# HansBambel/SmaAt-UNet

Hardware: NVIDIA H100
Metric: SmaAt-UNet fwd frames/sec @ B=32 12×288×288; depthwise % HBM roofline (higher is better)
Workload: dtype f32

## Files before the change

### include/smaat_b200.h

```cpp
#ifndef SMAAT_B200_H_
#define SMAAT_B200_H_

#include <stddef.h>
#include <stdint.h>

#ifdef __cplusplus
extern "C" {
#endif

#define SMAAT_ABI_VERSION 3

#define SMAAT_OK 0
#define SMAAT_E_BADARG (-1)
#define SMAAT_E_CUDA (-2)
#define SMAAT_E_UNSUPPORTED (-3)

#define SMAAT_PW_FP32_SIMT 0
#define SMAAT_PW_TF32 1
#define SMAAT_PW_TF32X3 2
#define SMAAT_PW_BF16 3

int smaat_abi_version(void);
const char* smaat_last_error(void);
uint64_t smaat_launch_count(void);
// ... 24 lines not shown
int smaat_dsconv_classify_eligible(const float* x0, int C0, int64_t x0_bstride, const float* x1, int C1, int64_t x1_bstride,
                                   const float* pw_w, int H, int W, int k, int Cout, int K, int mode);
int smaat_dsconv_classify_fwd(const float* x0, int C0, int64_t x0_bstride, const float* x1, int C1, int64_t x1_bstride,
                              const float* dw_w, const float* dw_b, const float* pw_w, const float* pw_w_lo,
                              const float* scale, const float* shift, const float* oc_w, const float* oc_b, int K,
                              float* logits, int64_t* classes, int B, int H, int W, int k, int Cout, int relu, int mode, void* stream);

int smaat_dsconv_cbam_eligible(const float* x0, int C0, int64_t x0_bstride, const float* x1, int C1, int64_t x1_bstride,
                               const float* pw_w, int H, int W, int k, int Cout, int mode, int with_gate, int with_pools);
int smaat_dsconv_pool_parts(int H, int W);
int smaat_dsconv_cbam_fwd(const float* x0, int C0, int64_t x0_bstride, const float* x1, int C1, int64_t x1_bstride,
                          const float* dw_w, const float* dw_b, const float* pw_w, const float* pw_w_lo,
                          const float* scale, const float* shift, float* y, int64_t y_bstride,
                          const float* gate_sc, const float* gate_sa, float* pool_sum, float* pool_max, float* pooled,
                          int B, int H, int W, int k, int Cout, int relu, int mode, void* stream);
int smaat_dsconv_maxpool_eligible(const float* x0, int C0, int64_t x0_bstride, const float* x1, int C1, int64_t x1_bstride,
                                  const float* pw_w, int H, int W, int k, int Cout, int mode);
int smaat_dsconv_maxpool_fwd(const float* x0, int C0, int64_t x0_bstride, const float* x1, int C1, int64_t x1_bstride,
                             const float* dw_w, const float* dw_b, const float* pw_w, const float* pw_w_lo,
                             const float* scale, const float* shift, float* y, int64_t y_bstride, float* pooled,
                             int B, int H, int W, int k, int Cout, int relu, int mode, void* stream);

int smaat_set_dsconv_impl(int impl);

int smaat_pw1x1_tc_eligible(const float* x, const float* w, int K, int Cout, int P);

int smaat_split_tf32(const float* src, float* hi, float* lo, int64_t n, void* stream);
int smaat_pack_bf16(const float* w, uint16_t* out, int rows, int cols, int cols_out, void* stream);

int smaat_bn_fold(const float* gamma, const float* beta, const float* rm, const float* rv,
                  const float* conv_bias, float eps, float* scale, float* shift, int C, void* stream);

int smaat_channel_stats(const float* x, double* stats, int B, int C, int P, void* stream);
int smaat_bn_finalize(const double* stats, double count, const float* gamma, const float* beta, float eps, float momentum,
                      float* running_mean, float* running_var, float* scale, float* shift,
                      float* mean_out, float* invstd_out, long long* num_batches_tracked, int C, void* stream);
int smaat_affine_act_fwd(const float* x, const float* scale, const float* shift, float* y,
                         int B, int C, int P, int act, void* stream);

int smaat_maxpool2_fwd(const float* x, float* y, int64_t N, int H, int W, void* stream);

int smaat_upsample2x_pad_fwd(const float* x, float* y, int64_t y_bstride,
                             int B, int C, int H, int W, int Ho, int Wo, void* stream);

int smaat_cbam_pool_fwd(const float* x, float* avg, float* mx, int64_t N, int P, void* stream);
int smaat_cbam_pool_maxpool_fwd(const float* x, float* avg, float* mx, float* pooled, int64_t N, int H, int W, void* stream);
// ... 129 lines not shown
```

### smaat_unet_b200/_lib.py

```python
from __future__ import annotations

import ctypes as C
import os

_HERE = os.path.dirname(os.path.abspath(__file__))
LIB_PATH = os.path.join(_HERE, "libsmaat_b200.so")

_p = C.c_void_p
_i = C.c_int
_l = C.c_int64
_f = C.c_float

SIGNATURES = {
    "smaat_dw3x3_fwd": [_p, _i, _l, _p, _i, _l, _p, _p, _p, _p, _p, _i, _i, _i, _i, _i, _p],
    "smaat_pw1x1_fwd": [_p, _p, _p, _p, _p, _p, _l, _p, _i, _i, _i, _i, _i, _i, _p],
    "smaat_pw1x1_tc_eligible": [_p, _p, _i, _i, _i],
    "smaat_dsconv_eligible": [_p, _i, _l, _p, _i, _l, _p, _i, _i, _i, _i],
    "smaat_dsconv_eligible2": [_p, _i, _l, _p, _i, _l, _p, _i, _i, _i, _i, _i],
    "smaat_set_dsconv_impl": [_i],
    "smaat_dsconv_fwd": [_p, _i, _l, _p, _i, _l, _p, _p, _p, _p, _p, _p, _p, _l, _p, _i, _i, _i, _i, _i, _i, _i, _p],
    "smaat_dsconv_outconv_fwd": [_p, _i, _l, _p, _i, _l, _p, _p, _p, _p, _p, _p, _p, _p, _p, _i, _i, _i, _i, _i, _i, _i, _p],
    "smaat_dsconv_classify_eligible": [_p, _i, _l, _p, _i, _l, _p, _i, _i, _i, _i, _i, _i],
    "smaat_dsconv_classify_fwd": [_p, _i, _l, _p, _i, _l, _p, _p, _p, _p, _p, _p, _p, _p, _i, _p, _p, _i, _i, _i, _i, _i, _i, _i, _p],
    "smaat_dsconv_cbam_eligible": [_p, _i, _l, _p, _i, _l, _p, _i, _i, _i, _i, _i, _i, _i],
    "smaat_dsconv_pool_parts": [_i, _i],
    "smaat_dsconv_maxpool_eligible": [_p, _i, _l, _p, _i, _l, _p, _i, _i, _i, _i, _i],
    "smaat_dsconv_maxpool_fwd": [_p, _i, _l, _p, _i, _l, _p, _p, _p, _p, _p, _p, _p, _l, _p, _i, _i, _i, _i, _i, _i, _i, _p],
    "smaat_dsconv_cbam_fwd": [_p, _i, _l, _p, _i, _l, _p, _p, _p, _p, _p, _p, _p, _l, _p, _p, _p, _p, _p, _i, _i, _i, _i, _i, _i, _i, _p],
    "smaat_split_tf32": [_p, _p, _p, _l, _p],
    "smaat_pack_bf16": [_p, _p, _i, _i, _i, _p],
    "smaat_bn_fold": [_p, _p, _p, _p, _p, _f, _p, _p, _i, _p],
    "smaat_channel_stats": [_p, _p, _i, _i, _i, _p],
    "smaat_bn_finalize": [_p, C.c_double, _p, _p, _f, _f, _p, _p, _p, _p, _p, _p, _p, _i, _p],
    "smaat_affine_act_fwd": [_p, _p, _p, _p, _i, _i, _i, _i, _p],
    "smaat_maxpool2_fwd": [_p, _p, _l, _i, _i, _p],
    "smaat_upsample2x_pad_fwd": [_p, _p, _l, _i, _i, _i, _i, _i, _i, _p],
    "smaat_cbam_pool_fwd": [_p, _p, _p, _l, _i, _p],
    "smaat_cbam_pool_maxpool_fwd": [_p, _p, _p, _p, _l, _i, _i, _p],
    "smaat_cbam_mlp_fwd": [_p, _p, _p, _p, _p, _p, _p, _i, _i, _i, _p],
    "smaat_cbam_reduce_fwd": [_p, _p, _p, _i, _i, _i, _p],
    "smaat_cbam_gate_fwd": [_p, _p, _p, _p, _p, _i, _i, _i, _i, _p],
    "smaat_cbam_scale_fwd": [_p, _p, _p, _p, _l, _i, _i, _i, _p],
# ... 94 lines not shown
```

### smaat_unet_b200/csrc/dsconv_fused.cu

```cuda
#include <stdlib.h>

#include <type_traits>

#include "tc_common.cuh"

namespace smaat {

struct DsParams {
  const float* dw_w;
  const float* dw_b;
  const float* scale;
  const float* shift;
  float* y;
  int64_t y_bstride;
  double* stats;
  const float* oc_w;
  const float* oc_b;
  float* oc_y;
  const float* gate_sc;
  float* pool_sum;
  float* pool_max;
  float* pooled;
  int pooled_bf16;
  int npart;
  int ncls;
  int64_t* cls;
  int C0, C1, H, W, Cout, relu, K;
  int tiles_x, tiles_y, npass, total_tiles, nchunks;
};

constexpr int DS_MAX_CLASSES = 32;

template <int N_TILE, int KPL, int PW, Prec P, bool A_SMEM, typename TA = float>
struct DsCfg {
  static constexpr bool X3 = P == Prec::TF32X3;
  static constexpr int ESZ = (int)sizeof(TA);
  static_assert(ESZ == 4 || (P == Prec::BF16 && KPL != 4), "bf16 activations: the bf16 register-form instances, k = 1, 2");
  static_assert(P != Prec::BF16 || !A_SMEM, "BF16: register A form only");
  static constexpr int PH = TC_BM / PW;
  static constexpr int XM = 16 / ESZ;
  static constexpr int BW = PW + 2 * XM, BH = PH + 2;
  static constexpr int CC = TC_BK / KPL;
  static constexpr int IN_BYTES = CC * BH * BW * ESZ;
  static constexpr int A_BYTES = TC_BM * TC_BK * 4;
  static constexpr int B_BYTES = N_TILE * TC_BK * (P == Prec::BF16 ? 2 : 4);
  static constexpr int AST_BYTES = (X3 && A_SMEM ? 2 : 1) * A_BYTES;
  static constexpr int BST_BYTES = (X3 ? 2 : 1) * B_BYTES;
  static constexpr int OFF_ALO = A_BYTES;
  static constexpr int OFF_BLO = B_BYTES;
  static constexpr int NG = N_TILE > 64 ? 1 : 2;
  static constexpr int AS = X3 ? (A_SMEM ? (N_TILE > 64 ? 2 : 3) : 2 + NG) : 4;
  static constexpr int BS = X3 ? (A_SMEM && N_TILE > 64 ? 2 : 3) : 4;
  static constexpr int AFF_N = 512;
  static constexpr int BAR_BYTES = 512;
  static constexpr int FREE = 224 * 1024 - 1024 - BAR_BYTES - 3 * AFF_N * 4 - AS * AST_BYTES - BS * BST_BYTES;
  static constexpr int ST_BOX = 32 * 64 * ESZ;
  static constexpr int ST_WANT = 2;
  static constexpr int ST_BUFS = (FREE - 2 * ST_WANT * ST_BOX) / IN_BYTES >= 2 ? ST_WANT
                                 : (FREE - 2 * ST_BOX) / IN_BYTES >= 2     ? 1
                                                                           : 0;
  static constexpr int ST_BYTES = 2 * ST_BUFS * ST_BOX;
  static_assert(ST_BUFS > 0 || (FREE - 2 * ST_BOX) / IN_BYTES < 2, "staging falls back only where one buffer does not fit");
  static constexpr int SA_TX = BH * BW * 4;
  static constexpr int SA_BYTES = (SA_TX + 127) / 128 * 128;
  static constexpr int CLS_MIN = 21 * (N_TILE + 1) * 4;
  static constexpr int RING_CLS = (FREE - ST_BYTES + 3 * 1024 - CLS_MIN) / 1024 * 1024;
  static constexpr int IS_FIT = (RING_CLS < FREE - ST_BYTES ? RING_CLS : FREE - ST_BYTES) / (IN_BYTES + SA_BYTES);
  static constexpr int IS = IS_FIT > 8 ? 8 : IS_FIT;
  static_assert(IS * (IN_BYTES + SA_BYTES) + ST_BYTES <= FREE, "gate boxes fit beside the input ring");
  static constexpr int OFF_SA = IS * IN_BYTES;
  static constexpr int OFF_A = ((OFF_SA + IS * SA_BYTES + 1023) / 1024) * 1024;
  static constexpr int OFF_BR = OFF_A + AS * AST_BYTES;
  static constexpr int OFF_ST = OFF_BR + BS * BST_BYTES;
  static constexpr int OFF_BAR = OFF_ST + ST_BYTES;
  static_assert((IS * NG + IS + 2 * AS + 2 * BS) * 8 <= BAR_BYTES, "barrier block");
  static constexpr int TOTAL = OFF_BAR + BAR_BYTES + 3 * AFF_N * 4 + 1024;
  static constexpr int OFF_CLS = OFF_BAR + BAR_BYTES + 3 * AFF_N * 4;
  static constexpr int CLS_FIT = (227 * 1024 - TOTAL) / ((N_TILE + 1) * 4);
  static constexpr int MAX_CLASSES = CLS_FIT < DS_MAX_CLASSES ? CLS_FIT : DS_MAX_CLASSES;
  static constexpr int CLS_SMEM = MAX_CLASSES * (N_TILE + 1) * 4;
  static_assert(MAX_CLASSES >= 21, "the class weights of a 21-class model fit beside the rings");
  static_assert(TOTAL + CLS_SMEM <= 227 * 1024, "the class weights take no shared memory from the rings");
  static constexpr uint32_t B_TX = BST_BYTES;
  static constexpr int PROD_WARP = 12;
  static constexpr int THREADS = 384 + 128 * NG;
  static constexpr int REGS_LAUNCH = (65536 / THREADS) / 8 * 8;
  static constexpr int REGS_TMA = 24;
  static constexpr int REGS_PROD = N_TILE > 64 ? 104 : REGS_LAUNCH;
  static constexpr int REGS_MMA = ((THREADS / 128 * REGS_LAUNCH - REGS_TMA - NG * REGS_PROD) / 2) / 8 * 8;
  static constexpr int REGS_SUM = REGS_TMA + 2 * REGS_MMA + NG * REGS_PROD;
  static_assert(REGS_SUM <= THREADS / 128 * REGS_LAUNCH && REGS_MMA >= REGS_LAUNCH, "register budget");
  static constexpr int KS = (X3 && N_TILE == 64) ? 2 : TC_BK / 8;
  static_assert(IS >= 2, "input ring");
  static_assert(NG <= AS, "phase-parity barriers");
  static_assert(IN_BYTES % 128 == 0, "TMA destination alignment");
  static_assert(TOTAL <= 227 * 1024, "shared memory budget");
};

__device__ __forceinline__ void tma_store_4d(const CUtensorMap* m, uint32_t src, int c0, int c1, int c2, int c3) {
  asm volatile("cp.async.bulk.tensor.4d.global.shared::cta.bulk_group [%0, {%2, %3, %4, %5}], [%1];" ::"l"(
                   reinterpret_cast<uint64_t>(m)),
               "r"(src), "r"(c0), "r"(c1), "r"(c2), "r"(c3)
               : "memory");
}
__device__ __forceinline__ void bulk_commit() { asm volatile("cp.async.bulk.commit_group;" ::: "memory"); }
template <int N>
__device__ __forceinline__ void bulk_wait_read() { asm volatile("cp.async.bulk.wait_group.read %0;" ::"n"(N) : "memory"); }
__device__ __forceinline__ void bulk_wait_all() { asm volatile("cp.async.bulk.wait_group 0;" ::: "memory"); }
__device__ __forceinline__ void wg_sync(int id) { asm volatile("bar.sync %0, 128;" ::"r"(id) : "memory"); }

__device__ __forceinline__ void quad_transpose(float (&v)[4], int q) {
  const bool h1 = q & 2, h0 = q & 1;
#pragma unroll
  for (int e = 0; e < 2; ++e) {
    const float r = __shfl_xor_sync(0xffffffffu, h1 ? v[e] : v[e + 2], 8);
    if (h1) v[e] = r; else v[e + 2] = r;
  }
#pragma unroll
  for (int e = 0; e < 4; e += 2) {
    const float r = __shfl_xor_sync(0xffffffffu, h0 ? v[e] : v[e + 1], 4);
    if (h0) v[e] = r; else v[e + 1] = r;
  }
}

template <int N_TILE, int KPL, int PW, Prec PREC, bool A_SMEM, typename TA = float>
__device__ __forceinline__ void dsconv_body(const CUtensorMap& map_in0, const CUtensorMap& map_in1, const CUtensorMap& map_w,
                                            const CUtensorMap& map_wlo, const CUtensorMap& map_y, const CUtensorMap& map_sa,
                                            const DsParams& p) {
  using L = DsCfg<N_TILE, KPL, PW, PREC, A_SMEM, TA>;
  constexpr bool X3 = L::X3;
  constexpr bool BA = L::ESZ == 2;
  constexpr int PH = L::PH, BW = L::BW, BH = L::BH, CC = L::CC, IS = L::IS, AS = L::AS, BS = L::BS;
  extern __shared__ __align__(1024) unsigned char smem_dyn[];
  unsigned char* smem = smem_dyn + ((1024u - (smem_u32(smem_dyn) & 1023u)) & 1023u);
  unsigned char* a_base = smem + L::OFF_A;
  unsigned char* b_base = smem + L::OFF_BR;
  uint64_t* bars = reinterpret_cast<uint64_t*>(smem + L::OFF_BAR);
  uint64_t* in_full = bars;
  uint64_t* in_empty = in_full + IS * L::NG;
  uint64_t* a_full = in_empty + IS;
  uint64_t* a_empty = a_full + AS;
  uint64_t* b_full = a_empty + AS;
  uint64_t* b_empty = b_full + BS;
  float* aff = reinterpret_cast<float*>(smem + L::OFF_BAR + L::BAR_BYTES);

  const int warp = __shfl_sync(0xffffffffu, (int)(threadIdx.x >> 5), 0);
  const int lane = threadIdx.x & 31;
  const int nch = p.nchunks;
  const int tiles_per_img = p.tiles_x * p.tiles_y * p.npass;
  auto decode = [&](int tile, int& b, int& ty, int& tx, int& np) {
    b = tile / tiles_per_img;
    int t2 = tile - b * tiles_per_img;
    np = t2 % p.npass;
    t2 /= p.npass;
    ty = t2 / p.tiles_x;
    tx = t2 - ty * p.tiles_x;
  };

  if (warp == 0 && lane == 0) {
    tma_prefetch_desc(&map_in0);
    tma_prefetch_desc(&map_in1);
    tma_prefetch_desc(&map_w);
    if (X3) tma_prefetch_desc(&map_wlo);
    if (L::ST_BUFS && !p.oc_y) tma_prefetch_desc(&map_y);
    if (p.gate_sc) tma_prefetch_desc(&map_sa);
    for (int s = 0; s < IS; ++s) {
      for (int g = 0; g < L::NG; ++g) mbar_init(&in_full[s * L::NG + g], 1);
      mbar_init(&in_empty[s], 128);
    }
    for (int s = 0; s < AS; ++s) {
      mbar_init(&a_full[s], 128);
      mbar_init(&a_empty[s], 8);
    }
    for (int s = 0; s < BS; ++s) {
      mbar_init(&b_full[s], 1);
      mbar_init(&b_empty[s], 8);
    }
    fence_barrier_init();
  }
  for (int c = threadIdx.x; c < L::AFF_N; c += blockDim.x) {
    aff[c] = (c < p.Cout && p.scale) ? __ldg(p.scale + c) : 1.f;
    aff[L::AFF_N + c] = (c < p.Cout && p.shift) ? __ldg(p.shift + c) : 0.f;
    aff[2 * L::AFF_N + c] = (c < p.Cout && p.oc_w) ? __ldg(p.oc_w + c) : 0.f;
  }
  float* cls_w = reinterpret_cast<float*>(smem + L::OFF_CLS);
  float* cls_b = cls_w + L::MAX_CLASSES * N_TILE;
  if (p.ncls) {
    for (int i = threadIdx.x; i < p.ncls * N_TILE; i += blockDim.x) {
      const int cl = i / N_TILE, c = i - cl * N_TILE;
      cls_w[i] = c < p.Cout ? __ldg(p.oc_w + (int64_t)cl * p.Cout + c) : 0.f;
    }
    for (int cl = threadIdx.x; cl < p.ncls; cl += blockDim.x) cls_b[cl] = p.oc_b ? __ldg(p.oc_b + cl) : 0.f;
  }
  __syncthreads();

  if (warp < 4) {
    regs_dealloc<L::REGS_TMA>();
    if (warp == 0 && lane == 0) {
      uint32_t gc = 0;
      for (int tile = blockIdx.x; tile < p.total_tiles; tile += gridDim.x) {
        int b, ty, tx, np;
        decode(tile, b, ty, tx, np);
        const int x0 = tx * PW, y0 = ty * PH;
        for (int i = 0; i < nch; ++i, ++gc) {
          const int s = gc % IS;
          mbar_wait(&in_empty[s], ((gc / IS) & 1u) ^ 1u);
          uint64_t* full = &in_full[s * L::NG + (int)(gc % (uint32_t)L::NG)];
          const int cb = i * CC;
          const bool gated = p.gate_sc && cb < p.C0;
          mbar_arrive_expect_tx(full, L::IN_BYTES + (gated ? L::SA_TX : 0));
          if (gated) tma_load_3d(smem + L::OFF_SA + s * L::SA_BYTES, &map_sa, full, x0 - L::XM, y0 - 1, b);
          const CUtensorMap* m = (cb < p.C0) ? &map_in0 : &map_in1;
          const int cc = (cb < p.C0) ? cb : cb - p.C0;
          asm volatile(
              "cp.async.bulk.tensor.4d.shared::cluster.global.mbarrier::complete_tx::bytes [%0], [%1, {%3, %4, %5, %6}], [%2];" ::
                  "r"(smem_u32(smem + s * L::IN_BYTES)),
              "l"(reinterpret_cast<uint64_t>(m)), "r"(smem_u32(full)), "r"(x0 - L::XM), "r"(y0 - 1), "r"(cc), "r"(b)
              : "memory");
        }
      }
    }
    if (warp == 1 && lane == 0) {
      uint32_t gc = 0;
      for (int tile = blockIdx.x; tile < p.total_tiles; tile += gridDim.x) {
        int b, ty, tx, np;
        decode(tile, b, ty, tx, np);
        for (int i = 0; i < nch; ++i, ++gc) {
          const int sb = gc % BS;
          mbar_wait(&b_empty[sb], ((gc / BS) & 1u) ^ 1u);
          mbar_arrive_expect_tx(&b_full[sb], L::B_TX);
// ... 13 lines not shown
    const int m1 = A_SMEM ? m0 + 8 : tc_row_pixel(wg, wq, 1, g);
    const float act_lo = p.relu ? 0.f : -INFINITY;
    const int64_t P = (int64_t)p.H * p.W;
    constexpr int SW_MASK = PW == 32 ? 7 : 3;
    const int quad = g & 3, slot = quad ^ (t & 2);
    const int st_ch = 2 * t + (slot & 1);
    const int st_px = ((slot & 2) ? m1 : m0) - quad - 64 * wg;
    const uint32_t st_a0 = (uint32_t)(st_ch * 64 * L::ESZ + st_px * L::ESZ);
    const uint32_t st_off = BA ? st_a0 : st_a0 ^ (((st_a0 >> 7) & SW_MASK) << 4);
    const uint32_t st_base = smem_u32(smem + L::OFF_ST) + (uint32_t)(wg * L::ST_BUFS * L::ST_BOX);
    const bool st_leader = (threadIdx.x & 127) == 0;
    uint32_t st_n = 0;
    uint32_t gc = 0;
    for (int tile = blockIdx.x; tile < p.total_tiles; tile += gridDim.x) {
      int b, ty, tx, np;
      decode(tile, b, ty, tx, np);
      float acc[N_TILE / 2];
#pragma unroll
      for (int i = 0; i < N_TILE / 2; ++i) acc[i] = 0.f;
      auto release = [&](uint32_t c) {
        __syncwarp();
        if (lane == 0) {
          mbar_arrive(&a_empty[c % AS]);
          mbar_arrive(&b_empty[c % BS]);
        }
      };
      auto wait_stages = [&](const unsigned char*& ast, uint64_t& bd, uint64_t& bl) {
        const int sa = gc % AS, sb = gc % BS;
        mbar_wait(&a_full[sa], (gc / AS) & 1u);
        mbar_wait(&b_full[sb], (gc / BS) & 1u);
        ast = a_base + sa * L::AST_BYTES;
        bd = make_b_desc<PREC>(smem_u32(b_base + sb * L::BST_BYTES));
        bl = make_kmajor_desc(smem_u32(b_base + sb * L::BST_BYTES + L::OFF_BLO));
      };
      if (A_SMEM) {
        for (int i = 0; i < nch; ++i, ++gc) {
          const unsigned char* ast;
          uint64_t bd0, bl0;
          wait_stages(ast, bd0, bl0);
          const uint32_t a_addr = smem_u32(ast) + (uint32_t)(wg * 64 * 128);
          const uint64_t ad0 = make_kmajor_desc(a_addr), al0 = make_kmajor_desc(a_addr + L::OFF_ALO);
          wgmma_fence();
#pragma unroll
          for (int kk = 0; kk < TC_BK / 8; ++kk) {
            Wgmma<N_TILE>::ss(acc, ad0 + (uint64_t)(2 * kk), bd0 + (uint64_t)(2 * kk), 1u);
            if (X3) {
// ... 232 lines not shown
              if (v1) st_act(yc + o1, fmaxf(fmaf(acc[4 * j + 2 + e], sc, sh), act_lo));
            }
          }
        }
      }
    }
    if (L::ST_BUFS && st_leader) bulk_wait_all();
    return;
  }

  {
    if (L::REGS_PROD < L::REGS_LAUNCH) regs_dealloc<L::REGS_PROD>();
    const int g = (warp - L::PROD_WARP) >> 2;
    const int t = threadIdx.x - 32 * L::PROD_WARP - 128 * g;
    const int Cin = p.C0 + p.C1;
    constexpr int KH = KPL == 4 ? 2 : KPL, NT = CC * 8;
    const int kr0 = KH == KPL ? 0 : t / NT * KH;
    const float* dw_w = p.dw_w + kr0 * 9;
    const float* dw_b = p.dw_b ? p.dw_b + kr0 : nullptr;
    uint32_t gc = 0, iph = 0;
    for (int tile = blockIdx.x; tile < p.total_tiles; tile += gridDim.x) {
      const int b = tile / tiles_per_img;
      for (int i = 0; i < nch; ++i, ++gc) {
        if ((int)(gc % (uint32_t)L::NG) != g) continue;
        const int s = gc % IS;
        const bool gated = p.gate_sc && i * CC < p.C0;
        auto task_base = [&](int task) { return KH == KPL ? task : task & (NT - 1); };
        float wr[KH][9], br[KH], gsc = 0.f;
        auto task_channel = [&](int task) { return (PW == 32) ? (task >> 3) : (((task >> 4) << 1) | ((task >> 2) & 1)); };
        auto load_weights = [&](int task) {
          const int gch = i * CC + task_channel(task_base(task));
          const bool chv = gch < Cin;
#pragma unroll
          for (int kk = 0; kk < KH; ++kk) {
            const int gk = gch * KPL + kk;
#pragma unroll
            for (int w9 = 0; w9 < 9; ++w9) wr[kk][w9] = chv ? __ldg(dw_w + (int64_t)gk * 9 + w9) : 0.f;
            br[kk] = (chv && dw_b) ? __ldg(dw_b + gk) : 0.f;
          }
          if (gated) gsc = gch < p.C0 ? __ldg(p.gate_sc + (int64_t)b * p.C0 + gch) : 0.f;
        };
        load_weights(t);
        mbar_wait(&in_full[s * L::NG + g], (iph >> s) & 1u);
        iph ^= 1u << s;
        const int sa = gc % AS;
        mbar_wait(&a_empty[sa], ((gc / AS) & 1u) ^ 1u);
        unsigned char* my_op = a_base + sa * L::AST_BYTES;
        const TA* in_stage = reinterpret_cast<const TA*>(smem + s * L::IN_BYTES);
// ... 56 lines not shown
                  a = fmaf(wr[kk][0], w0[j], a); a = fmaf(wr[kk][1], w0[j + 1], a); a = fmaf(wr[kk][2], w0[j + 2], a);
                  a = fmaf(wr[kk][3], w1[j], a); a = fmaf(wr[kk][4], w1[j + 1], a); a = fmaf(wr[kk][5], w1[j + 2], a);
                  a = fmaf(wr[kk][6], w2[j], a); a = fmaf(wr[kk][7], w2[j + 1], a); a = fmaf(wr[kk][8], w2[j + 2], a);
                  o4[j] = a;
                }
                if (A_SMEM) {
                  const int kr = ci * KPL + kr0 + kk;
#pragma unroll
                  for (int j = 0; j < 4; ++j) {
                    const uint32_t off = kmajor_offset(m + j, kr);
                    const float h = X3 ? tf32_hi(o4[j]) : o4[j];
                    *reinterpret_cast<float*>(my_op + off) = h;
                    if (X3) *reinterpret_cast<float*>(my_op + L::OFF_ALO + off) = o4[j] - h;
                  }
                  continue;
                }
                *reinterpret_cast<float4*>(my_op + a_tile_offset(ci * KPL + kr0 + kk, m)) = make_float4(o4[0], o4[1], o4[2], o4[3]);
              }
            }
          }
        };
        if (gated) stencil(std::true_type{}); else stencil(std::false_type{});
        if (A_SMEM) fence_proxy_async_smem();
        mbar_arrive(&a_full[sa]);
        mbar_arrive(&in_empty[s]);
      }
    }
  }
}

__host__ __device__ constexpr Prec tf32_prec(bool x3) { return x3 ? Prec::TF32X3 : Prec::TF32; }

template <int N_TILE, int KPL, int PW, bool X3, bool A_SMEM>
__global__ void __launch_bounds__(DsCfg<N_TILE, KPL, PW, tf32_prec(X3), A_SMEM>::THREADS, 1)
    dsconv_fused_kernel(const __grid_constant__ CUtensorMap map_in0, const __grid_constant__ CUtensorMap map_in1,
                        const __grid_constant__ CUtensorMap map_w, const __grid_constant__ CUtensorMap map_wlo,
                        const __grid_constant__ CUtensorMap map_y, const __grid_constant__ CUtensorMap map_sa,
                        const DsParams p) {
  dsconv_body<N_TILE, KPL, PW, tf32_prec(X3), A_SMEM>(map_in0, map_in1, map_w, map_wlo, map_y, map_sa, p);
}

template <int N_TILE, int PW, bool X3>
__global__ void __launch_bounds__(DsCfg<N_TILE, 4, PW, tf32_prec(X3), false>::THREADS, 1)
    dsconv_kpl4_kernel(const __grid_constant__ CUtensorMap map_in0, const __grid_constant__ CUtensorMap map_in1,
                       const __grid_constant__ CUtensorMap map_w, const __grid_constant__ CUtensorMap map_wlo,
                       const __grid_constant__ CUtensorMap map_y, const __grid_constant__ CUtensorMap map_sa,
                       const DsParams p) {
  dsconv_body<N_TILE, 4, PW, tf32_prec(X3), false>(map_in0, map_in1, map_w, map_wlo, map_y, map_sa, p);
}

template <int N_TILE, int KPL, int PW>
__global__ void __launch_bounds__(DsCfg<N_TILE, KPL, PW, Prec::BF16, false>::THREADS, 1)
    dsconv_bf16_kernel(const __grid_constant__ CUtensorMap map_in0, const __grid_constant__ CUtensorMap map_in1,
                       const __grid_constant__ CUtensorMap map_w, const __grid_constant__ CUtensorMap map_wlo,
                       const __grid_constant__ CUtensorMap map_y, const __grid_constant__ CUtensorMap map_sa,
                       const DsParams p) {
  dsconv_body<N_TILE, KPL, PW, Prec::BF16, false>(map_in0, map_in1, map_w, map_wlo, map_y, map_sa, p);
}

template <int N_TILE, int KPL, int PW>
__global__ void __launch_bounds__(DsCfg<N_TILE, KPL, PW, Prec::BF16, false, uint16_t>::THREADS, 1)
    dsconv_bf16act_kernel(const __grid_constant__ CUtensorMap map_in0, const __grid_constant__ CUtensorMap map_in1,
                          const __grid_constant__ CUtensorMap map_w, const __grid_constant__ CUtensorMap map_wlo,
                          const __grid_constant__ CUtensorMap map_y, const __grid_constant__ CUtensorMap map_sa,
                          const DsParams p) {
  dsconv_body<N_TILE, KPL, PW, Prec::BF16, false, uint16_t>(map_in0, map_in1, map_w, map_wlo, map_y, map_sa, p);
}

template <int N_TILE, int KPL, int PW, Prec P, bool A_SMEM, typename TA = float>
static auto ds_kernel() {
  static_assert(KPL == 1 || KPL == 2 || (KPL == 4 && !A_SMEM), "fused DS conv instances: k = 1, 2 (both A forms), 4 (register form)");
  if constexpr (sizeof(TA) == 2) return dsconv_bf16act_kernel<N_TILE, KPL, PW>;
  else if constexpr (P == Prec::BF16) return dsconv_bf16_kernel<N_TILE, KPL, PW>;
  else if constexpr (KPL == 4) return dsconv_kpl4_kernel<N_TILE, PW, P == Prec::TF32X3>;
  else return dsconv_fused_kernel<N_TILE, KPL, PW, P == Prec::TF32X3, A_SMEM>;
}

template <int N_TILE, int KPL, int PW, Prec P, bool A_SMEM, typename TA = float>
static int launch_ds(const CUtensorMap& m0, const CUtensorMap& m1, const CUtensorMap& mw, const CUtensorMap& mwl,
                     const CUtensorMap& my, const CUtensorMap& msa, DsParams p, int B, cudaStream_t st) {
  using L = DsCfg<N_TILE, KPL, PW, P, A_SMEM, TA>;
  auto kern = ds_kernel<N_TILE, KPL, PW, P, A_SMEM, TA>();
  if (p.pooled && !L::ST_BUFS) return fail(SMAAT_E_UNSUPPORTED, "dsconv: the CBAM pools and the max-pool need the staged epilogue");
  if (p.ncls > L::MAX_CLASSES)
    return fail(SMAAT_E_UNSUPPORTED, "dsconv+classify: %d classes, this instance keeps the weights of at most %d", p.ncls, L::MAX_CLASSES);
  static std::atomic<uint64_t> attr_mask{0};
  if (first_use_on_device(attr_mask)) {
    cudaError_t e = cudaFuncSetAttribute(kern, cudaFuncAttributeMaxDynamicSharedMemorySize, L::TOTAL + L::CLS_SMEM);
    if (e != cudaSuccess)
      return fail(SMAAT_E_CUDA, "dsconv: smem attribute (%d B): %s", L::TOTAL + L::CLS_SMEM, cudaGetErrorString(e));
    int r = check_reg_budget((const void*)kern, L::THREADS, L::REGS_SUM, "dsconv");
    if (r) return r;
  }
  p.tiles_x = ceil_div(p.W, PW);
  p.tiles_y = ceil_div(p.H, L::PH);
  p.npass = ceil_div(p.Cout, N_TILE);
  const int64_t total = (int64_t)B * p.tiles_x * p.tiles_y * p.npass;
  SMAAT_REQUIRE(total < (1ll << 31), "dsconv: too many tiles");
  p.total_tiles = (int)total;
  p.nchunks = ceil_div(p.C0 + p.C1, L::CC);
  p.npart = 2 * p.tiles_x * p.tiles_y;
  const int grid = p.total_tiles < num_sms() ? p.total_tiles : num_sms();
  kern<<<grid, L::THREADS, L::TOTAL + (p.ncls ? L::CLS_SMEM : 0), st>>>(m0, m1, mw, mwl, my, msa, p);
  SMAAT_LAUNCH_CHECK("smaat_dsconv_fwd");
  return SMAAT_OK;
}

static int pick_pw(int H, int W) {
  double best = 1e9;
  int pw = 0;
  const int cand[2] = {32, 16};
  for (int i = 0; i < 2; ++i) {
    const int c = cand[i], ph = TC_BM / c;
    const double waste = ((double)ceil_div(W, c) * c / W) * ((double)ceil_div(H, ph) * ph / H);
    if (waste < best - 1e-9) {
      best = waste;
      pw = c;
    }
  }
  return best <= 1.35 ? pw : 0;
}

static int ds_impl();

static bool ds_eligible(const float* x0, int C0, int64_t bs0, const float* x1, int C1, int64_t bs1, const float* pw_w,
                        const float* pw_w_lo, const float* y, int64_t y_bstride, int H, int W, int k, int Cout, bool stats,
                        bool outconv, bool bf16 = false, bool bact = false) {
  if (k != 1 && k != 2 && !(k == 4 && ds_impl() != 1)) return false;
// ... 41 lines not shown
}

static std::atomic<int> g_ds_impl{-1};
static int ds_impl() {
  int v = g_ds_impl.load(std::memory_order_relaxed);
  if (v < 0) {
    const char* e = getenv("SMAAT_DS_IMPL");
    v = e ? atoi(e) : 0;
    if (v < 0 || v > 2) v = 0;
    g_ds_impl.store(v, std::memory_order_relaxed);
  }
  return v;
}

}

using namespace smaat;

extern "C" int smaat_set_dsconv_impl(int impl) {
  SMAAT_REQUIRE(impl >= 0 && impl <= 2, "set_dsconv_impl: 0 = auto, 1 = A operand from shared memory, 2 = A operand from registers");
  g_ds_impl.store(impl, std::memory_order_relaxed);
  return SMAAT_OK;
}

extern "C" int smaat_dsconv_eligible2(const float* x0, int C0, int64_t x0_bstride, const float* x1, int C1, int64_t x1_bstride,
                                      const float* pw_w, int H, int W, int k, int Cout, int with_stats) {
  return ds_eligible(x0, C0, x0_bstride, x1, C1, x1_bstride, pw_w, nullptr, nullptr, 0, H, W, k, Cout, with_stats != 0, false) ? 1
                                                                                                                                : 0;
}

extern "C" int smaat_dsconv_eligible(const float* x0, int C0, int64_t x0_bstride, const float* x1, int C1, int64_t x1_bstride,
                                     const float* pw_w, int H, int W, int k, int Cout) {
  return smaat_dsconv_eligible2(x0, C0, x0_bstride, x1, C1, x1_bstride, pw_w, H, W, k, Cout, 0);
}

extern "C" int smaat_dsconv_cbam_eligible(const float* x0, int C0, int64_t x0_bstride, const float* x1, int C1, int64_t x1_bstride,
                                          const float* pw_w, int H, int W, int k, int Cout, int mode, int with_gate, int with_pools) {
  if (mode != SMAAT_PW_TF32 && mode != SMAAT_PW_TF32X3 && mode != SMAAT_PW_BF16) return 0;
  if (!ds_eligible(x0, C0, x0_bstride, x1, C1, x1_bstride, pw_w, nullptr, nullptr, 0, H, W, k, Cout, false, false,
                   mode == SMAAT_PW_BF16))
    return 0;
  (void)with_gate;
  if (with_pools && !ds_staged(Cout > 64 ? 128 : 64, k, pick_pw(H, W), mode, ds_impl() == 1)) return 0;
  return 1;
}

// ... 93 lines not shown
    const uint64_t str[3] = {0, (uint64_t)W * 4, (uint64_t)H * W * 4};
    const uint32_t sbox[3] = {(uint32_t)(pw + 2 * xm), (uint32_t)(ph + 2), 1u};
    int r = make_tmap_f32(&msa, gate_sa, 3, dims, str, sbox, CU_TENSOR_MAP_SWIZZLE_NONE, "dsconv(gate sa)");
    if (r) return r;
  }
  DsParams p;
  p.dw_w = dw_w; p.dw_b = dw_b; p.scale = scale; p.shift = shift; p.y = y; p.y_bstride = y_bstride; p.stats = stats;
  p.oc_w = oc_w; p.oc_b = oc_b; p.oc_y = oc_y; p.ncls = ncls; p.cls = cls;
  p.gate_sc = gate_sc; p.pool_sum = pool_sum; p.pool_max = pool_max; p.pooled = pooled; p.pooled_bf16 = pooled_bf16; p.npart = 0;
  p.C0 = C0; p.C1 = C1; p.H = H; p.W = W; p.Cout = Cout; p.relu = relu; p.K = K;
  p.tiles_x = p.tiles_y = p.npass = p.total_tiles = p.nchunks = 0;

#define DS_DISPATCH(NT, KP, PWv)                                                                           \
  if (bact) return launch_ds<NT, KP, PWv, Prec::BF16, false, uint16_t>(m0, m1, mw, mwl, my, msa, p, B, st);         \
  if (bf16) return launch_ds<NT, KP, PWv, Prec::BF16, false>(m0, m1, mw, mwl, my, msa, p, B, st);                    \
  return x3 ? (a_smem ? launch_ds<NT, KP, PWv, Prec::TF32X3, true>(m0, m1, mw, mwl, my, msa, p, B, st)               \
                      : launch_ds<NT, KP, PWv, Prec::TF32X3, false>(m0, m1, mw, mwl, my, msa, p, B, st))             \
            : (a_smem ? launch_ds<NT, KP, PWv, Prec::TF32, true>(m0, m1, mw, mwl, my, msa, p, B, st)                 \
                      : launch_ds<NT, KP, PWv, Prec::TF32, false>(m0, m1, mw, mwl, my, msa, p, B, st))
#define DS_DISPATCH4(NT, PWv)                                                                                  \
  if (bf16) return launch_ds<NT, 4, PWv, Prec::BF16, false>(m0, m1, mw, mwl, my, msa, p, B, st);                  \
  return x3 ? launch_ds<NT, 4, PWv, Prec::TF32X3, false>(m0, m1, mw, mwl, my, msa, p, B, st)                  \
            : launch_ds<NT, 4, PWv, Prec::TF32, false>(m0, m1, mw, mwl, my, msa, p, B, st)
  if (n_tile == 64) {
    if (k == 4)      { if (pw == 32) { DS_DISPATCH4(64, 32); } else { DS_DISPATCH4(64, 16); } }
    else if (k == 2) { if (pw == 32) { DS_DISPATCH(64, 2, 32); } else { DS_DISPATCH(64, 2, 16); } }
    else             { if (pw == 32) { DS_DISPATCH(64, 1, 32); } else { DS_DISPATCH(64, 1, 16); } }
  } else {
    if (k == 4)      { if (pw == 32) { DS_DISPATCH4(128, 32); } else { DS_DISPATCH4(128, 16); } }
    else if (k == 2) { if (pw == 32) { DS_DISPATCH(128, 2, 32); } else { DS_DISPATCH(128, 2, 16); } }
    else             { if (pw == 32) { DS_DISPATCH(128, 1, 32); } else { DS_DISPATCH(128, 1, 16); } }
  }
#undef DS_DISPATCH4
#undef DS_DISPATCH
}

extern "C" int smaat_dsconv_fwd(const float* x0, int C0, int64_t x0_bstride, const float* x1, int C1, int64_t x1_bstride,
                                const float* dw_w, const float* dw_b, const float* pw_w, const float* pw_w_lo,
                                const float* scale, const float* shift, float* y, int64_t y_bstride, double* stats, int B, int H,
                                int W, int k, int Cout, int relu, int mode, void* stream) {
  SMAAT_REQUIRE(y, "dsconv: null output");
  return dsconv_run(x0, C0, x0_bstride, x1, C1, x1_bstride, dw_w, dw_b, pw_w, pw_w_lo, scale, shift, y, y_bstride, stats, nullptr,
                    nullptr, nullptr, 0, nullptr, nullptr, nullptr, nullptr, nullptr, nullptr, B, H, W, k, Cout, relu, mode, stream);
}

extern "C" int smaat_dsconv_outconv_fwd(const float* x0, int C0, int64_t x0_bstride, const float* x1, int C1, int64_t x1_bstride,
                                        const float* dw_w, const float* dw_b, const float* pw_w, const float* pw_w_lo,
                                        const float* scale, const float* shift, const float* oc_w, const float* oc_b,
                                        float* logits, int B, int H, int W, int k, int Cout, int relu, int mode, void* stream) {
  SMAAT_REQUIRE(oc_w && logits, "dsconv+outconv: null pointer");
  return dsconv_run(x0, C0, x0_bstride, x1, C1, x1_bstride, dw_w, dw_b, pw_w, pw_w_lo, scale, shift, nullptr, 0, nullptr, oc_w, oc_b,
                    logits, 0, nullptr, nullptr, nullptr, nullptr, nullptr, nullptr, B, H, W, k, Cout, relu, mode, stream);
}

extern "C" int smaat_dsconv_classify_eligible(const float* x0, int C0, int64_t x0_bstride, const float* x1, int C1, int64_t x1_bstride,
// ... 117 lines not shown
```

### smaat_unet_b200/ops.py

```python
from __future__ import annotations

import contextlib
import ctypes as C
import gc
import os

import torch

from . import _lib

PW_MODES = {"fp32": 0, "tf32": 1, "tf32x3": 2, "bf16": 3}
_pw_mode = os.environ.get("SMAAT_PW_MODE", "tf32x3")
assert _pw_mode in PW_MODES, f"SMAAT_PW_MODE must be one of {list(PW_MODES)}"


def set_pointwise_mode(mode: str) -> None:
    global _pw_mode
    if mode not in PW_MODES:
        raise ValueError(f"pointwise mode must be one of {list(PW_MODES)}")
    _pw_mode = mode


def get_pointwise_mode() -> str:
    return _pw_mode
# ... 167 lines not shown
        ybs = Cout * P
    else:
        out, ybs = _nchw_bstride(out, "out")
    mode = mode or _pw_mode
    m = PW_MODES[mode]
    if m != 0 and (not tc_eligible(x, w2d) or (Cout > 512 and (scale is not None or shift is not None))):
        m = 0
    w2d, wlo = weight_operands(w2d, m, w_split)
    _call(f"smaat_pw1x1_fwd[K{K}_N{Cout}_P{P}]", 4 * B * P * (K + Cout) + 4 * K * Cout, 2 * B * P * K * Cout, _lib.load().smaat_pw1x1_fwd, _ptr(x), _ptr(w2d), _ptr(wlo), _ptr(scale), _ptr(shift), _ptr(out), ybs, _ptr(stats),
                                           B, K, Cout, P, int(bool(relu)), m, _stream())
    return out


_fuse_ds = os.environ.get("SMAAT_FUSE_DS", "1") != "0"


def set_fused_dsconv(enabled: bool) -> None:
    global _fuse_ds
    _fuse_ds = bool(enabled)


def set_dsconv_impl(impl: str) -> None:
    _lib.check(_lib.load().smaat_set_dsconv_impl({"auto": 0, "smem": 1, "regs": 2}[impl]), "smaat_set_dsconv_impl")


def dsconv_takes(x, x1, pw_weight, k, mode=None, stats=False) -> bool:
    mode = mode or _pw_mode
    if not _fuse_ds or PW_MODES[mode] == 0:
        return False
    x, bs0, x1, C1, bs1 = _concat_operands(x, x1)
    w2d = _pw_matrix(pw_weight)
    lib = _lib.load()
    args = (_ptr(x), x.shape[1], bs0, _ptr(x1), C1, bs1, _ptr(w2d), x.shape[2], x.shape[3], k, w2d.shape[0])
    if not lib.smaat_dsconv_eligible2(*args, int(bool(stats))):
        return False
    return PW_MODES[mode] != 3 or bool(lib.smaat_dsconv_cbam_eligible(*args, 3, 0, 0))


def dsconv_cbam_takes(x, x1, pw_weight, k, gate=False, pools=False, mode=None) -> bool:
    mode = mode or _pw_mode
    if not _fuse_ds or PW_MODES[mode] == 0:
        return False
    x, bs0, x1, C1, bs1 = _concat_operands(x, x1)
    w2d = _pw_matrix(pw_weight)
    return bool(_lib.load().smaat_dsconv_cbam_eligible(_ptr(x), x.shape[1], bs0, _ptr(x1), C1, bs1, _ptr(w2d), x.shape[2], x.shape[3], k,
                                                       w2d.shape[0], PW_MODES[mode], int(bool(gate)), int(bool(pools))))
# ... 645 lines not shown
```

Before: 2709.

## Split depthwise stencil work across 2-CTA clusters sharing A tiles via DSMEM

Measured after the change: 2767, median of 6. +2.1%, better.

```diff
diff --git a/include/smaat_b200.h b/include/smaat_b200.h
--- a/include/smaat_b200.h
+++ b/include/smaat_b200.h
@@ -70,6 +70,9 @@
                              int B, int H, int W, int k, int Cout, int relu, int mode, void* stream);
 
 int smaat_set_dsconv_impl(int impl);
+
+int smaat_set_dsconv_pair(int on);
+int smaat_dsconv_pair_clusters(void);
 
 int smaat_pw1x1_tc_eligible(const float* x, const float* w, int K, int Cout, int P);
 
diff --git a/smaat_unet_b200/_lib.py b/smaat_unet_b200/_lib.py
--- a/smaat_unet_b200/_lib.py
+++ b/smaat_unet_b200/_lib.py
@@ -18,6 +18,8 @@
     "smaat_dsconv_eligible": [_p, _i, _l, _p, _i, _l, _p, _i, _i, _i, _i],
     "smaat_dsconv_eligible2": [_p, _i, _l, _p, _i, _l, _p, _i, _i, _i, _i, _i],
     "smaat_set_dsconv_impl": [_i],
+    "smaat_set_dsconv_pair": [_i],
+    "smaat_dsconv_pair_clusters": [],
     "smaat_dsconv_fwd": [_p, _i, _l, _p, _i, _l, _p, _p, _p, _p, _p, _p, _p, _l, _p, _i, _i, _i, _i, _i, _i, _i, _p],
     "smaat_dsconv_outconv_fwd": [_p, _i, _l, _p, _i, _l, _p, _p, _p, _p, _p, _p, _p, _p, _p, _i, _i, _i, _i, _i, _i, _i, _p],
     "smaat_dsconv_classify_eligible": [_p, _i, _l, _p, _i, _l, _p, _i, _i, _i, _i, _i, _i],
diff --git a/smaat_unet_b200/csrc/dsconv_fused.cu b/smaat_unet_b200/csrc/dsconv_fused.cu
--- a/smaat_unet_b200/csrc/dsconv_fused.cu
+++ b/smaat_unet_b200/csrc/dsconv_fused.cu
@@ -31,7 +31,7 @@
 
 constexpr int DS_MAX_CLASSES = 32;
 
-template <int N_TILE, int KPL, int PW, Prec P, bool A_SMEM, typename TA = float>
+template <int N_TILE, int KPL, int PW, Prec P, bool A_SMEM, typename TA = float, int CL = 1>
 struct DsCfg {
   static constexpr bool X3 = P == Prec::TF32X3;
   static constexpr int ESZ = (int)sizeof(TA);
@@ -49,7 +49,7 @@
   static constexpr int OFF_ALO = A_BYTES;
   static constexpr int OFF_BLO = B_BYTES;
   static constexpr int NG = N_TILE > 64 ? 1 : 2;
-  static constexpr int AS = X3 ? (A_SMEM ? (N_TILE > 64 ? 2 : 3) : 2 + NG) : 4;
+  static constexpr int AS = X3 ? (A_SMEM ? (N_TILE > 64 ? 2 : 3) : 2 + (CL > 1 && KPL == 2 ? CL : 1) * NG) : 4;
   static constexpr int BS = X3 ? (A_SMEM && N_TILE > 64 ? 2 : 3) : 4;
   static constexpr int AFF_N = 512;
   static constexpr int BAR_BYTES = 512;
@@ -93,6 +93,7 @@
   static constexpr int KS = (X3 && N_TILE == 64) ? 2 : TC_BK / 8;
   static_assert(IS >= 2, "input ring");
   static_assert(NG <= AS, "phase-parity barriers");
+  static constexpr bool PAIRABLE = N_TILE == 128 && !A_SMEM && ESZ == 4 && KPL != 4 && P != Prec::BF16 && 2 * NG <= AS;
   static_assert(IN_BYTES % 128 == 0, "TMA destination alignment");
   static_assert(TOTAL <= 227 * 1024, "shared memory budget");
 };
@@ -109,6 +110,31 @@
 __device__ __forceinline__ void bulk_wait_all() { asm volatile("cp.async.bulk.wait_group 0;" ::: "memory"); }
 __device__ __forceinline__ void wg_sync(int id) { asm volatile("bar.sync %0, 128;" ::"r"(id) : "memory"); }
 
+__device__ __forceinline__ uint32_t cluster_rank() {
+  uint32_t r;
+  asm volatile("mov.u32 %0, %%cluster_ctarank;" : "=r"(r));
+  return r;
+}
+__device__ __forceinline__ void cluster_sync() {
+  asm volatile("barrier.cluster.arrive.release;\n\tbarrier.cluster.wait.acquire;" ::: "memory");
+}
+__device__ __forceinline__ uint32_t cluster_addr(uint32_t a, uint32_t rank) {
+  uint32_t r;
+  asm volatile("mapa.shared::cluster.u32 %0, %1, %2;" : "=r"(r) : "r"(a), "r"(rank));
+  return r;
+}
+__device__ __forceinline__ void mbar_arrive_remote(uint32_t bar) {
+  asm volatile("mbarrier.arrive.shared::cluster.b64 _, [%0];" ::"r"(bar) : "memory");
+}
+__device__ __forceinline__ void mbar_arrive_expect_tx_remote(uint32_t bar, uint32_t bytes) {
+  asm volatile("mbarrier.arrive.expect_tx.shared::cluster.b64 _, [%0], %1;" ::"r"(bar), "r"(bytes) : "memory");
+}
+__device__ __forceinline__ void bulk_copy_to_peer(uint32_t dst, uint32_t src, uint32_t bytes, uint32_t bar) {
+  asm volatile("cp.async.bulk.shared::cluster.shared::cta.mbarrier::complete_tx::bytes [%0], [%1], %2, [%3];" ::"r"(dst), "r"(src),
+               "r"(bytes), "r"(bar)
+               : "memory");
+}
+
 __device__ __forceinline__ void quad_transpose(float (&v)[4], int q) {
   const bool h1 = q & 2, h0 = q & 1;
 #pragma unroll
@@ -123,11 +149,12 @@
   }
 }
 
-template <int N_TILE, int KPL, int PW, Prec PREC, bool A_SMEM, typename TA = float>
+template <int N_TILE, int KPL, int PW, Prec PREC, bool A_SMEM, typename TA = float, int CL = 1>
 __device__ __forceinline__ void dsconv_body(const CUtensorMap& map_in0, const CUtensorMap& map_in1, const CUtensorMap& map_w,
                                             const CUtensorMap& map_wlo, const CUtensorMap& map_y, const CUtensorMap& map_sa,
                                             const DsParams& p) {
-  using L = DsCfg<N_TILE, KPL, PW, PREC, A_SMEM, TA>;
+  using L = DsCfg<N_TILE, KPL, PW, PREC, A_SMEM, TA, CL>;
+  static_assert(CL == 1 || (CL == 2 && L::PAIRABLE), "CTA pairs: the N_TILE 128 register-form fp32 instances, k = 1, 2");
   constexpr bool X3 = L::X3;
   constexpr bool BA = L::ESZ == 2;
   constexpr int PH = L::PH, BW = L::BW, BH = L::BH, CC = L::CC, IS = L::IS, AS = L::AS, BS = L::BS;
@@ -147,6 +174,7 @@
   const int warp = __shfl_sync(0xffffffffu, (int)(threadIdx.x >> 5), 0);
   const int lane = threadIdx.x & 31;
   const int nch = p.nchunks;
+  const uint32_t rank = CL > 1 ? cluster_rank() : 0u, peer = rank ^ 1u;
   const int tiles_per_img = p.tiles_x * p.tiles_y * p.npass;
   auto decode = [&](int tile, int& b, int& ty, int& tx, int& np) {
     b = tile / tiles_per_img;
@@ -169,8 +197,8 @@
       mbar_init(&in_empty[s], 128);
     }
     for (int s = 0; s < AS; ++s) {
-      mbar_init(&a_full[s], 128);
-      mbar_init(&a_empty[s], 8);
+      mbar_init(&a_full[s], CL > 1 ? 1 : 128);
+      mbar_init(&a_empty[s], 8 * CL);
     }
     for (int s = 0; s < BS; ++s) {
       mbar_init(&b_full[s], 1);
@@ -193,6 +221,7 @@
     for (int cl = threadIdx.x; cl < p.ncls; cl += blockDim.x) cls_b[cl] = p.oc_b ? __ldg(p.oc_b + cl) : 0.f;
   }
   __syncthreads();
+  if (CL > 1) cluster_sync();
 
   if (warp < 4) {
     regs_dealloc<L::REGS_TMA>();
@@ -203,9 +232,11 @@
         decode(tile, b, ty, tx, np);
         const int x0 = tx * PW, y0 = ty * PH;
         for (int i = 0; i < nch; ++i, ++gc) {
-          const int s = gc % IS;
-          mbar_wait(&in_empty[s], ((gc / IS) & 1u) ^ 1u);
-          uint64_t* full = &in_full[s * L::NG + (int)(gc % (uint32_t)L::NG)];
+          if (CL > 1 && gc % CL != rank) continue;
+          const uint32_t f = gc / CL;
+          const int s = f % IS;
+          mbar_wait(&in_empty[s], ((f / IS) & 1u) ^ 1u);
+          uint64_t* full = &in_full[s * L::NG + (int)(f % (uint32_t)L::NG)];
           const int cb = i * CC;
           const bool gated = p.gate_sc && cb < p.C0;
           mbar_arrive_expect_tx(full, L::IN_BYTES + (gated ? L::SA_TX : 0));
@@ -265,6 +296,7 @@
         __syncwarp();
         if (lane == 0) {
           mbar_arrive(&a_empty[c % AS]);
+          if (CL > 1) mbar_arrive_remote(cluster_addr(smem_u32(&a_empty[c % AS]), peer));
           mbar_arrive(&b_empty[c % BS]);
         }
       };
@@ -543,8 +575,10 @@
     for (int tile = blockIdx.x; tile < p.total_tiles; tile += gridDim.x) {
       const int b = tile / tiles_per_img;
       for (int i = 0; i < nch; ++i, ++gc) {
-        if ((int)(gc % (uint32_t)L::NG) != g) continue;
-        const int s = gc % IS;
+        if (CL > 1 && gc % CL != rank) continue;
+        const uint32_t f = gc / CL;
+        if ((int)(f % (uint32_t)L::NG) != g) continue;
+        const int s = f % IS;
         const bool gated = p.gate_sc && i * CC < p.C0;
         auto task_base = [&](int task) { return KH == KPL ? task : task & (NT - 1); };
         float wr[KH][9], br[KH], gsc = 0.f;
@@ -647,7 +681,18 @@
         };
         if (gated) stencil(std::true_type{}); else stencil(std::false_type{});
         if (A_SMEM) fence_proxy_async_smem();
-        mbar_arrive(&a_full[sa]);
+        if constexpr (CL > 1) {
+          fence_proxy_async_smem();
+          asm volatile("bar.sync 4, 128;" ::: "memory");
+          if (t == 0) {
+            mbar_arrive(&a_full[sa]);
+            const uint32_t rbar = cluster_addr(smem_u32(&a_full[sa]), peer);
+            mbar_arrive_expect_tx_remote(rbar, L::A_BYTES);
+            bulk_copy_to_peer(cluster_addr(smem_u32(my_op), peer), smem_u32(my_op), L::A_BYTES, rbar);
+          }
+        } else {
+          mbar_arrive(&a_full[sa]);
+        }
         mbar_arrive(&in_empty[s]);
       }
     }
@@ -665,6 +710,16 @@
   dsconv_body<N_TILE, KPL, PW, tf32_prec(X3), A_SMEM>(map_in0, map_in1, map_w, map_wlo, map_y, map_sa, p);
 }
 
+template <int KPL, int PW, bool X3>
+__global__ void __launch_bounds__(DsCfg<128, KPL, PW, tf32_prec(X3), false>::THREADS, 1)
+    dsconv_pair_kernel(const __grid_constant__ CUtensorMap map_in0, const __grid_constant__ CUtensorMap map_in1,
+                       const __grid_constant__ CUtensorMap map_w, const __grid_constant__ CUtensorMap map_wlo,
+                       const __grid_constant__ CUtensorMap map_y, const __grid_constant__ CUtensorMap map_sa,
+                       const DsParams p) {
+  dsconv_body<128, KPL, PW, tf32_prec(X3), false, float, 2>(map_in0, map_in1, map_w, map_wlo, map_y, map_sa, p);
+  cluster_sync();
+}
+
 template <int N_TILE, int PW, bool X3>
 __global__ void __launch_bounds__(DsCfg<N_TILE, 4, PW, tf32_prec(X3), false>::THREADS, 1)
     dsconv_kpl4_kernel(const __grid_constant__ CUtensorMap map_in0, const __grid_constant__ CUtensorMap map_in1,
@@ -692,20 +747,23 @@
   dsconv_body<N_TILE, KPL, PW, Prec::BF16, false, uint16_t>(map_in0, map_in1, map_w, map_wlo, map_y, map_sa, p);
 }
 
-template <int N_TILE, int KPL, int PW, Prec P, bool A_SMEM, typename TA = float>
+template <int N_TILE, int KPL, int PW, Prec P, bool A_SMEM, typename TA = float, int CL = 1>
 static auto ds_kernel() {
   static_assert(KPL == 1 || KPL == 2 || (KPL == 4 && !A_SMEM), "fused DS conv instances: k = 1, 2 (both A forms), 4 (register form)");
-  if constexpr (sizeof(TA) == 2) return dsconv_bf16act_kernel<N_TILE, KPL, PW>;
+  if constexpr (CL == 2) return dsconv_pair_kernel<KPL, PW, P == Prec::TF32X3>;
+  else if constexpr (sizeof(TA) == 2) return dsconv_bf16act_kernel<N_TILE, KPL, PW>;
   else if constexpr (P == Prec::BF16) return dsconv_bf16_kernel<N_TILE, KPL, PW>;
   else if constexpr (KPL == 4) return dsconv_kpl4_kernel<N_TILE, PW, P == Prec::TF32X3>;
   else return dsconv_fused_kernel<N_TILE, KPL, PW, P == Prec::TF32X3, A_SMEM>;
 }
 
-template <int N_TILE, int KPL, int PW, Prec P, bool A_SMEM, typename TA = float>
+static std::atomic<int> g_ds_pairs_resident{0};
+
+template <int N_TILE, int KPL, int PW, Prec P, bool A_SMEM, typename TA = float, int CL = 1>
 static int launch_ds(const CUtensorMap& m0, const CUtensorMap& m1, const CUtensorMap& mw, const CUtensorMap& mwl,
                      const CUtensorMap& my, const CUtensorMap& msa, DsParams p, int B, cudaStream_t st) {
-  using L = DsCfg<N_TILE, KPL, PW, P, A_SMEM, TA>;
-  auto kern = ds_kernel<N_TILE, KPL, PW, P, A_SMEM, TA>();
+  using L = DsCfg<N_TILE, KPL, PW, P, A_SMEM, TA, CL>;
+  auto kern = ds_kernel<N_TILE, KPL, PW, P, A_SMEM, TA, CL>();
   if (p.pooled && !L::ST_BUFS) return fail(SMAAT_E_UNSUPPORTED, "dsconv: the CBAM pools and the max-pool need the staged epilogue");
   if (p.ncls > L::MAX_CLASSES)
     return fail(SMAAT_E_UNSUPPORTED, "dsconv+classify: %d classes, this instance keeps the weights of at most %d", p.ncls, L::MAX_CLASSES);
@@ -725,10 +783,54 @@
   p.total_tiles = (int)total;
   p.nchunks = ceil_div(p.C0 + p.C1, L::CC);
   p.npart = 2 * p.tiles_x * p.tiles_y;
+  if constexpr (CL == 2) {
+    SMAAT_REQUIRE(p.npass == 2 && !p.ncls, "dsconv: CTA pairs take two 128-channel passes and no head");
+    cudaLaunchAttribute attr[1];
+    attr[0].id = cudaLaunchAttributeClusterDimension;
+    attr[0].val.clusterDim.x = 2;
+    attr[0].val.clusterDim.y = 1;
+    attr[0].val.clusterDim.z = 1;
+    cudaLaunchConfig_t cfg = {};
+    cfg.blockDim = dim3(L::THREADS);
+    cfg.dynamicSmemBytes = L::TOTAL;
+    cfg.stream = st;
+    cfg.attrs = attr;
+    cfg.numAttrs = 1;
+    static std::atomic<int> pairs[64];
+    int dev = 0;
+    cudaGetDevice(&dev);
+    int np = pairs[dev & 63].load(std::memory_order_relaxed);
+    if (np <= 0) {
+      cfg.gridDim = dim3(2 * (unsigned)num_sms());
+      cudaError_t e = cudaOccupancyMaxActiveClusters(&np, kern, &cfg);
+      if (e != cudaSuccess || np < 1)
+        return fail(SMAAT_E_CUDA, "dsconv: no resident CTA pair at %d B of shared memory: %s", L::TOTAL, cudaGetErrorString(e));
+      pairs[dev & 63].store(np, std::memory_order_relaxed);
+    }
+    g_ds_pairs_resident.store(np, std::memory_order_relaxed);
+    const int npatch = p.total_tiles / 2;
+    cfg.gridDim = dim3(2 * (unsigned)(npatch < np ? npatch : np));
+    cudaError_t e = cudaLaunchKernelEx(&cfg, kern, m0, m1, mw, mwl, my, msa, p);
+    if (e != cudaSuccess) return fail(SMAAT_E_CUDA, "smaat_dsconv_fwd (CTA pairs): %s", cudaGetErrorString(e));
+    SMAAT_LAUNCH_CHECK("smaat_dsconv_fwd");
+    return SMAAT_OK;
+  }
   const int grid = p.total_tiles < num_sms() ? p.total_tiles : num_sms();
   kern<<<grid, L::THREADS, L::TOTAL + (p.ncls ? L::CLS_SMEM : 0), st>>>(m0, m1, mw, mwl, my, msa, p);
   SMAAT_LAUNCH_CHECK("smaat_dsconv_fwd");
   return SMAAT_OK;
+}
+
+static std::atomic<int> g_ds_pair{-1};
+static bool ds_pair(bool x3, int k) {
+  int v = g_ds_pair.load(std::memory_order_relaxed);
+  if (v < 0) {
+    const char* e = getenv("SMAAT_DS_PAIR");
+    v = e ? atoi(e) : 2;
+    if (v < 0 || v > 2) v = 2;
+    g_ds_pair.store(v, std::memory_order_relaxed);
+  }
+  return v == 1 || (v == 2 && (!x3 || k == 2));
 }
 
 static int pick_pw(int H, int W) {
@@ -816,6 +918,14 @@
   g_ds_impl.store(impl, std::memory_order_relaxed);
   return SMAAT_OK;
 }
+
+extern "C" int smaat_set_dsconv_pair(int on) {
+  SMAAT_REQUIRE(on >= 0 && on <= 2, "set_dsconv_pair: 0 = one CTA per pass, 1 = CTA pairs, 2 = auto");
+  g_ds_pair.store(on, std::memory_order_relaxed);
+  return SMAAT_OK;
+}
+
+extern "C" int smaat_dsconv_pair_clusters(void) { return g_ds_pairs_resident.load(std::memory_order_relaxed); }
 
 extern "C" int smaat_dsconv_eligible2(const float* x0, int C0, int64_t x0_bstride, const float* x1, int C1, int64_t x1_bstride,
                                       const float* pw_w, int H, int W, int k, int Cout, int with_stats) {
@@ -955,15 +1065,20 @@
   if (bf16) return launch_ds<NT, 4, PWv, Prec::BF16, false>(m0, m1, mw, mwl, my, msa, p, B, st);                  \
   return x3 ? launch_ds<NT, 4, PWv, Prec::TF32X3, false>(m0, m1, mw, mwl, my, msa, p, B, st)                  \
             : launch_ds<NT, 4, PWv, Prec::TF32, false>(m0, m1, mw, mwl, my, msa, p, B, st)
+#define DS_DISPATCH_PAIR(KP, PWv)                                                                                  \
+  if (pair) return x3 ? launch_ds<128, KP, PWv, Prec::TF32X3, false, float, 2>(m0, m1, mw, mwl, my, msa, p, B, st) \
+                      : launch_ds<128, KP, PWv, Prec::TF32, false, float, 2>(m0, m1, mw, mwl, my, msa, p, B, st)
+  const bool pair = ds_pair(x3, k) && Cout == 256 && !bact && !bf16 && !a_smem && !head;
   if (n_tile == 64) {
     if (k == 4)      { if (pw == 32) { DS_DISPATCH4(64, 32); } else { DS_DISPATCH4(64, 16); } }
     else if (k == 2) { if (pw == 32) { DS_DISPATCH(64, 2, 32); } else { DS_DISPATCH(64, 2, 16); } }
     else             { if (pw == 32) { DS_DISPATCH(64, 1, 32); } else { DS_DISPATCH(64, 1, 16); } }
   } else {
     if (k == 4)      { if (pw == 32) { DS_DISPATCH4(128, 32); } else { DS_DISPATCH4(128, 16); } }
-    else if (k == 2) { if (pw == 32) { DS_DISPATCH(128, 2, 32); } else { DS_DISPATCH(128, 2, 16); } }
-    else             { if (pw == 32) { DS_DISPATCH(128, 1, 32); } else { DS_DISPATCH(128, 1, 16); } }
-  }
+    else if (k == 2) { if (pw == 32) { DS_DISPATCH_PAIR(2, 32); DS_DISPATCH(128, 2, 32); } else { DS_DISPATCH_PAIR(2, 16); DS_DISPATCH(128, 2, 16); } }
+    else             { if (pw == 32) { DS_DISPATCH_PAIR(1, 32); DS_DISPATCH(128, 1, 32); } else { DS_DISPATCH_PAIR(1, 16); DS_DISPATCH(128, 1, 16); } }
+  }
+#undef DS_DISPATCH_PAIR
 #undef DS_DISPATCH4
 #undef DS_DISPATCH
 }
diff --git a/smaat_unet_b200/ops.py b/smaat_unet_b200/ops.py
--- a/smaat_unet_b200/ops.py
+++ b/smaat_unet_b200/ops.py
@@ -213,6 +213,11 @@
 
 def set_dsconv_impl(impl: str) -> None:
     _lib.check(_lib.load().smaat_set_dsconv_impl({"auto": 0, "smem": 1, "regs": 2}[impl]), "smaat_set_dsconv_impl")
+
+
+def set_dsconv_pair(enabled) -> None:
+    v = 2 if enabled == "auto" else int(bool(enabled))
+    _lib.check(_lib.load().smaat_set_dsconv_pair(v), "smaat_set_dsconv_pair")
 
 
 def dsconv_takes(x, x1, pw_weight, k, mode=None, stats=False) -> bool:
```
